# aynik/carta1

Measured on AMD Instinct MI355X. Metric: atrac1_stereo_frames_per_s_encode, higher is better.
Workload: dtype f32+f64

## Files before the change

### carta1_amd/capi.py

```python
import ctypes as C
import os

HERE = os.path.dirname(os.path.abspath(__file__))
LIB_PATH = os.environ.get('C1_LIB') or os.path.join(HERE, 'lib', 'libcarta1_hip.so')

FRAME = 512
UNIT_BYTES = 212
SIGNAL_WHITE = 0
SIGNAL_PINK_BURSTS = 1
SIGNAL_MIXED = 2
SIGNAL_PARTIALS = 3


class Carta1Error(RuntimeError):
    def __init__(self, code, message):
        super().__init__('carta1_hip error %d: %s' % (code, message))
        self.code = code


class Tables(C.Structure):
    _fields_ = [('scale_factors', C.c_double * 64), ('window_short', C.c_double * 32),
                ('mdct_fwd64', C.c_double * 32), ('mdct_fwd256', C.c_double * 128),
                ('mdct_fwd512', C.c_double * 256), ('mdct_inv64', C.c_double * 32),
                ('mdct_inv256', C.c_double * 128), ('mdct_inv512', C.c_double * 256),
# ... 16 lines not shown
    'c1_ctx_destroy': (C.c_int, [C.c_void_p]),
    'c1_ctx_synchronize': (C.c_int, [C.c_void_p]),
    'c1_ctx_set_profiling': (C.c_int, [C.c_void_p, C.c_int]),
    'c1_ctx_kernel_ms': (C.c_int, [C.c_void_p, C.c_char_p, C.POINTER(C.c_double), C.POINTER(C.c_int)]),
    'c1_ctx_set_speculation': (C.c_int, [C.c_void_p, C.c_int]),
    'c1_ctx_set_decode_precision': (C.c_int, [C.c_void_p, C.c_int]),
    'c1_ctx_speculation_stats': (C.c_int, [C.c_void_p, C.POINTER(C.c_uint64), C.POINTER(C.c_uint64), C.c_int]),
    'c1_ctx_speculation_deferred': (C.c_int, [C.c_void_p, C.POINTER(C.c_uint64)]),
    'c1_ctx_quantization_stats': (C.c_int, [C.c_void_p, C.POINTER(C.c_uint64), C.POINTER(C.c_uint64)]),
    'c1_encode_device': (C.c_int, [C.c_void_p, C.POINTER(C.c_void_p), C.c_int, C.c_int64, C.c_int,
                                   C.POINTER(EncodeOptions), C.c_void_p]),
    'c1_encode_batch': (C.c_int, [C.c_void_p, C.POINTER(C.c_void_p), C.c_int, C.c_int64, C.c_int,
                                  C.POINTER(EncodeOptions), C.c_void_p]),
    'c1_encode_batch_multi': (C.c_int, [C.POINTER(C.c_int), C.c_int, C.POINTER(C.c_void_p), C.c_int, C.c_int64, C.c_int,
                                        C.POINTER(EncodeOptions), C.c_void_p]),
    'c1_decode_batch_multi': (C.c_int, [C.POINTER(C.c_int), C.c_int, C.c_void_p, C.c_int, C.c_int64, C.c_int,
                                        C.POINTER(C.c_void_p)]),
    'c1_decode_device': (C.c_int, [C.c_void_p, C.c_void_p, C.c_int, C.c_int64, C.c_int, C.POINTER(C.c_void_p)]),
    'c1_decode_batch': (C.c_int, [C.c_void_p, C.c_void_p, C.c_int, C.c_int64, C.c_int, C.POINTER(C.c_void_p)]),
    'c1_enc_stream_create': (C.c_int, [C.c_void_p, C.c_int, C.POINTER(EncodeOptions), C.POINTER(C.c_void_p)]),
    'c1_enc_stream_push': (C.c_int, [C.c_void_p, C.POINTER(C.c_void_p), C.c_int64, C.c_void_p]),
    'c1_enc_stream_destroy': (C.c_int, [C.c_void_p]),
    'c1_enc_stream_set_options': (C.c_int, [C.c_void_p, C.POINTER(EncodeOptions)]),
    'c1_dec_stream_create': (C.c_int, [C.c_void_p, C.c_int, C.POINTER(C.c_void_p)]),
    'c1_dec_stream_push': (C.c_int, [C.c_void_p, C.c_void_p, C.c_int64, C.POINTER(C.c_void_p)]),
    'c1_dec_stream_destroy': (C.c_int, [C.c_void_p]),
    'c1_generate_device': (C.c_int, [C.c_void_p, C.c_int, C.c_uint32, C.c_int64, C.c_void_p]),
    'c1_pcm_from_int_device': (C.c_int, [C.c_void_p, C.c_void_p, C.c_int, C.c_int, C.c_int64, C.POINTER(C.c_void_p)]),
    'c1_pcm_to_int16_device': (C.c_int, [C.c_void_p, C.POINTER(C.c_void_p), C.c_int, C.c_int64, C.c_void_p]),
    'c1_host_alloc': (C.c_int, [C.c_size_t, C.POINTER(C.c_void_p)]),
    'c1_host_free': (C.c_int, [C.c_void_p]),
    'c1_table_fast_paths': (C.c_int, [C.POINTER(C.c_int), C.POINTER(C.c_int)]),
    'c1_alloc_rank_form': (C.c_int, [C.POINTER(EncodeOptions), C.POINTER(C.c_int), C.POINTER(C.c_int)]),
    'c1_encode_wav_batch': (C.c_int, [C.c_void_p, C.c_void_p, C.c_int, C.c_int, C.c_int64, C.POINTER(EncodeOptions), C.c_void_p]),
    'c1_decode_wav16_batch': (C.c_int, [C.c_void_p, C.c_void_p, C.c_int, C.c_int64, C.c_void_p]),
    'c1_aea_header': (C.c_int, [C.c_char_p, C.c_uint32, C.c_int, C.c_void_p]),
    'c1_encode_stages_device': (C.c_int, [C.c_void_p, C.POINTER(C.c_void_p), C.c_int, C.c_int64, C.c_int,
                                          C.POINTER(EncodeOptions), C.c_void_p, C.c_void_p, C.c_void_p,
                                          C.c_void_p]),
    'c1_detect_stages_device': (C.c_int, [C.c_void_p, C.POINTER(C.c_void_p), C.c_int, C.c_int64, C.c_int,
                                          C.POINTER(EncodeOptions), C.c_void_p, C.c_void_p]),
    'c1_libm_device': (C.c_int, [C.c_void_p, C.c_int, C.c_void_p, C.c_void_p, C.c_int64]),
    'c1_detect_scores_device': (C.c_int, [C.c_void_p, C.POINTER(C.c_void_p), C.c_int, C.c_int64, C.c_int,
                                          C.POINTER(EncodeOptions), C.c_int, C.c_void_p, C.c_void_p, C.c_void_p]),
    'c1_detect_spec_mags_device': (C.c_int, [C.c_void_p, C.POINTER(C.c_void_p), C.c_int, C.c_int64, C.c_int, C.c_void_p, C.c_void_p]),
    'c1_log2f_error_device': (C.c_int, [C.c_void_p, C.c_uint32, C.c_uint64, C.POINTER(C.c_double)]),
    'c1_ctx_detection_stats': (C.c_int, [C.c_void_p, C.POINTER(C.c_uint64), C.POINTER(C.c_uint64)]),
    'c1_alloc_bounds_device': (C.c_int, [C.c_void_p, C.c_void_p, C.c_int64, C.c_void_p, C.c_void_p]),
    'c1_spec_stages_device': (C.c_int, [C.c_void_p, C.POINTER(C.c_void_p), C.c_int, C.c_int64, C.c_int,
                                        C.POINTER(EncodeOptions), C.c_void_p, C.c_void_p, C.c_void_p]),
    'c1_quantize': (C.c_int, [C.c_void_p, C.c_void_p, C.c_int, C.c_int, C.c_int, C.c_void_p]),
    'c1_dequantize': (C.c_int, [C.c_void_p, C.c_void_p, C.c_int, C.c_int, C.c_int, C.c_void_p]),
    'c1_fft': (C.c_int, [C.c_void_p, C.c_void_p, C.c_void_p, C.c_int, C.c_void_p]),
    'c1_qmf_analysis_batch': (C.c_int, [C.c_void_p, C.c_void_p, C.c_int64, C.c_int, C.c_void_p]),
    'c1_mdct_batch': (C.c_int, [C.c_void_p, C.c_void_p, C.c_int64, C.c_int, C.c_void_p, C.c_void_p, C.c_void_p]),
    'c1_unpack_units': (C.c_int, [C.c_void_p, C.c_void_p, C.c_int64, C.c_void_p, C.c_void_p, C.c_void_p, C.c_void_p, C.c_void_p]),
    'c1_dequantize_frames': (C.c_int, [C.c_void_p, C.c_int64, C.c_void_p, C.c_void_p, C.c_void_p, C.c_void_p, C.c_void_p, C.c_void_p]),
    'c1_imdct_batch': (C.c_int, [C.c_void_p, C.c_void_p, C.c_int64, C.c_int, C.c_void_p, C.c_void_p]),
    'c1_qmf_synthesis_batch': (C.c_int, [C.c_void_p, C.c_void_p, C.c_int64, C.c_int, C.c_void_p]),
    'c1_select_block_modes': (C.c_int, [C.c_void_p, C.c_void_p, C.c_int64, C.c_int, C.c_double, C.c_void_p]),
    'c1_quantize_frames': (C.c_int, [C.c_void_p, C.c_void_p, C.c_int64, C.c_void_p, C.c_void_p, C.c_void_p, C.c_void_p,
                                     C.c_void_p, C.c_void_p]),
    'c1_pack_units': (C.c_int, [C.c_void_p, C.c_int64, C.c_void_p, C.c_void_p, C.c_void_p, C.c_void_p, C.c_void_p, C.c_void_p]),
    'c1_decode_fields_device': (C.c_int, [C.c_void_p, C.c_int, C.c_int64, C.c_int, C.c_void_p, C.c_void_p, C.c_void_p, C.c_void_p,
                                          C.c_void_p, C.POINTER(C.c_void_p)]),
    'c1_decode_fields_batch': (C.c_int, [C.c_void_p, C.c_int, C.c_int64, C.c_int, C.c_void_p, C.c_void_p, C.c_void_p, C.c_void_p,
# ... 55 lines not shown
```

### carta1_amd/csrc/c1_api.hip

```cpp
#include <algorithm>
#include <cmath>
#include <cstdarg>
#include <cstdio>
#include <cstdlib>
#include <cstring>
#include <map>
#include <memory>
#include <atomic>
#include <mutex>
#include <string>
#include <thread>
#include <vector>

#include "c1_internal.h"
#include "c1_detect_bound.h"

#pragma clang fp contract(off)

namespace {

#include "c1_default_tables.inc"

thread_local std::string g_error;
int fail(int code, const char *fmt, ...) {
  char buf[512];
  va_list ap;
  va_start(ap, fmt);
  vsnprintf(buf, sizeof buf, fmt, ap);
  va_end(ap);
  g_error = buf;
  return code;
}
#define HIP_TRY(expr)                                                                        \
  do {                                                                                       \
    hipError_t e_ = (expr);                                                                  \
    if (e_ != hipSuccess) return fail(C1_ERR_HIP, "%s: %s", #expr, hipGetErrorString(e_)); \
  } while (0)

// ... 242 lines not shown
      const double dbits = (double)(b1 - b0);
      pri[s * 15 + wl] = (float)(d->biased[s] * ddf / dbits);
      uniq.push_back(pri[s * 15 + wl]);
    }
  std::sort(uniq.begin(), uniq.end());
  uniq.erase(std::unique(uniq.begin(), uniq.end()), uniq.end());
  for (int s = 1; s < 64; s++)
    for (int wl = 0; wl < 15; wl++) {
      const auto it = std::lower_bound(uniq.begin(), uniq.end(), pri[s * 15 + wl]);
      d->rank[s * 16 + wl] = (uint16_t)(1 + (it - uniq.begin()));
    }
  d->rank_affine = 0;
  {
    std::vector<int> order;
    for (int s = 1; s < 64; s++)
      for (int wl = 0; wl < 15; wl++) order.push_back(s * 16 + wl);
    std::sort(order.begin(), order.end(), [&](int x, int y) { return d->rank[x] < d->rank[y]; });
    for (int A = 1; A <= 12 && !d->rank_affine; A++)
      for (int B = 1; B <= 36 && !d->rank_affine; B++)
        for (int C = -2 * B; C <= 2 * B && !d->rank_affine; C++) {
          auto key = [&](int idx) { const int s = idx >> 4, wl = idx & 15; return wl == 0 ? A * s + C : A * s - B * wl - B; };
          bool ok = true;
          int lo = key(order[0]), hi = lo;
          for (size_t i = 1; i < order.size() && ok; i++) {
            const int k0 = key(order[i - 1]), k1 = key(order[i]);
            const bool req = d->rank[order[i]] == d->rank[order[i - 1]];
            if (req ? (k1 != k0) : !(k1 > k0)) ok = false;
            lo = std::min(lo, k1); hi = std::max(hi, k1);
          }
          if (ok && hi - lo + 1 < 1023) {
            d->rank_affine = 1; d->rank_a = A; d->rank_b = B; d->rank_c = C; d->rank_off = 1 - lo;
          }
        }
  }
  return C1_OK;
}

constexpr int kTotals = 8;
constexpr int64_t kSpecMinUnits = 64;
constexpr int kListHead = 8;
constexpr int64_t kMaxChunkFrames = (int64_t)1 << 27;

struct Timing {
  hipEvent_t start, stop;
  int kind;
};
enum { K_ANALYSIS = 0, K_ALLOCATE, K_PACK, K_DECODE, K_REDO, K_PACK_UNITS, K_DECODE_FIELDS, K_KINDS };
const char *const kKindNames[K_KINDS] = {"analysis", "allocate", "pack", "decode", "redo", "pack_units", "decode_fields"};

}

struct c1_ctx {
  std::recursive_mutex mu;
  int device = 0;
  hipStream_t stream = nullptr;
  bool own_stream = false;
  C1DevTables *d_tables = nullptr;
  C1DevEncOpts *d_opts = nullptr;
  c1_encode_options last_opts;
  bool have_opts = false;
  int64_t ws_units = 0;
  float *d_coefs[2] = {nullptr, nullptr};
  uint8_t *d_side[2] = {nullptr, nullptr};
  uint8_t *d_alloc[2] = {nullptr, nullptr};
  uint8_t *d_cand[2] = {nullptr, nullptr};
  uint32_t *d_work[2] = {nullptr, nullptr};
// ... 467 lines not shown
  if (!tables) { g_tables_custom = false; g_tables_gen++; return C1_OK; }
  const double *p = reinterpret_cast<const double *>(tables);
  for (size_t i = 0; i < sizeof(c1_tables) / sizeof(double); i++)
    if (!std::isfinite(p[i])) return fail(C1_ERR_ARG, "table entry %zu is not finite", i);
  g_tables = *tables;
  g_tables_custom = true;
  g_tables_gen++;
  return C1_OK;
}

int c1_table_fast_paths(int *scale_factor_bits, int *dequant_reciprocal) {
  c1_tables t;
  {
    std::lock_guard<std::mutex> lock(g_tables_mutex);
    if (g_tables_custom) t = g_tables; else default_tables(&t);
  }
  std::unique_ptr<C1DevTables> d(new C1DevTables);
  build_device_tables(t, d.get());
  if (scale_factor_bits) *scale_factor_bits = d->sf_fast;
  if (dequant_reciprocal) *dequant_reciprocal = d->dq_fast + d->dq_step;
  return C1_OK;
}

int c1_alloc_rank_form(const c1_encode_options *opts, int *affine, int *coef) {
  if (!opts) return fail(C1_ERR_ARG, "opts is NULL");
  std::unique_ptr<C1DevEncOpts> d(new C1DevEncOpts);
  const int rc = build_table_fields(*opts, d.get());
  if (rc) return rc;
  if (affine) *affine = d->rank_affine;
  if (coef) { coef[0] = d->rank_a; coef[1] = d->rank_b; coef[2] = d->rank_c; coef[3] = d->rank_off; }
  return C1_OK;
}

int c1_default_encode_options(c1_encode_options *out) {
  if (!out) return fail(C1_ERR_ARG, "out is NULL");
  memset(out, 0, sizeof *out);
  c1_tables t;
  {
    std::lock_guard<std::mutex> lock(g_tables_mutex);
    if (g_tables_custom) t = g_tables; else default_tables(&t);
  }
  memcpy(out->biased_scale_factors, t.scale_factors, sizeof out->biased_scale_factors);
  out->transient_threshold = 1.0;
  out->fixed_block_modes[0] = out->fixed_block_modes[1] = out->fixed_block_modes[2] = -1;
  return C1_OK;
}

int c1_ctx_create(int device, void *hip_stream, c1_ctx **out) {
  if (!out) return fail(C1_ERR_ARG, "out is NULL");
  *out = nullptr;
  int n = 0;
  const hipError_t e = hipGetDeviceCount(&n);
  if (e != hipSuccess || n == 0)
    return fail(C1_ERR_NO_DEVICE, "no HIP device available (%s); this library has no CPU path",
                e != hipSuccess ? hipGetErrorString(e) : "device count is 0");
  if (device < 0 || device >= n) return fail(C1_ERR_ARG, "device %d out of range (0..%d)", device, n - 1);
  HIP_TRY(hipSetDevice(device));
  c1_ctx *ctx = new c1_ctx();
  ctx->device = device;
  if (hip_stream) ctx->stream = (hipStream_t)hip_stream;
  else {
    const hipError_t se = hipStreamCreateWithFlags(&ctx->stream, hipStreamNonBlocking);
    if (se != hipSuccess) { delete ctx; return fail(C1_ERR_HIP, "hipStreamCreate: %s", hipGetErrorString(se)); }
    ctx->own_stream = true;
  }
  c1_tables t;
// ... 1930 lines not shown
```

### carta1_amd/csrc/c1_internal.h

```cpp
#pragma once

#include <hip/hip_runtime.h>
#include <stdint.h>
#include <stdlib.h>

#include "../../include/carta1_hip.h"

struct C1DevTables {
  double tap_e[24];
  double tap_o[24];
  double window[32];
  double mdct_fwd64[32];
  double mdct_fwd256[128];
  double mdct_fwd512[256];
  double mdct_inv64[32];
  double mdct_inv256[128];
  double mdct_inv512[256];
  double fft_tw[256][2];
  double scale_factors[64];
  double norm[64 * 16];
  double log1p10;
  uint32_t sf_m1, sf_m2;
  int32_t sf_fast;
  int32_t dq_fast;
  int32_t dq_step;
  double inv_range[16];
  float tap32[24];
  float tap_pair[26][2];
  float win32[32];
  float pre32_64[16][2];
  float pre32_256[64][2];
  float pre32_512[128][2];
  float r4b[4][3][2];
  float r4c[16][3][2];
  float r2d[64][2];
  float norm32[64 * 16];
  float inv32_64[16][2], inv32_256[64][2], inv32_512[128][2];
  float tw32[256][2];
  float spec_cz[4], spec_cw[4], spec_cl[4];
  float spec_cz_short[4], spec_cw_short[4], spec_cl_short[4];
  float spec_eabs;
  float det_ck[4];
  float det_eabs;
  int32_t spec_ok;
};

struct C1DevEncOpts {
  double biased[64];
  double threshold;
  int32_t modes[3];
  int32_t pad_;
  uint16_t rank[64 * 16];
  int32_t rank_affine, rank_a, rank_b, rank_c, rank_off;
  float la_slope, la_off;
  int32_t alloc_no_tonal;
};

constexpr int kRunFrames = 16;
constexpr int kRunFramesDecode = 64;
constexpr int kRunFramesLong = 64;
constexpr int kSideBytes = 64;
constexpr int kAllocBytes = 32;
constexpr int kCandidateBytes = 8 * 8 + 8 * 32 + 8 * 8;
constexpr int kCandLbOffset = 8 * 8 + 8 * 32;
constexpr int kEpsFloats = 4;
constexpr uint32_t kEpsFlagSfOpen = 1u;
constexpr uint32_t kEpsFlagExact = 2u;
constexpr int kSpecCheckFrames = 16;

struct C1EncodeLaunch {
  const float *pcm[C1_MAX_CHANNELS];
  int channels;
  int64_t frames;
  int halo_frames;
  const C1DevTables *tables;
  const C1DevEncOpts *opts;
  float *coefs;
  uint8_t *side;
  uint8_t *alloc;
  uint8_t *cand;
  uint32_t *work_list;
  uint32_t *work_count;
  uint32_t *sel_list;
  float *bands;
  float *mags;
  float *mag_bounds;
  uint8_t *units;
  float *eps;
  uint32_t *redo_list;
// ... 116 lines not shown
```

### carta1_amd/csrc/c1_k_allocate.hip

```cpp
#include "c1_device.h"

namespace {

constexpr int kHeapSlotsPerLane = 52 + 1;
constexpr uint32_t kLow = 0x1FFFFFu;
constexpr uint32_t kSentinel = 52u;
constexpr int kCandBytes = kCandidateBytes;
constexpr double kAlive = -1.0;

__device__ __forceinline__ uint32_t heap_entry(uint32_t rank, int size, int s, int wl, int b) {
  return (rank << 21) | ((uint32_t)size << 16) | ((uint32_t)s << 10) | ((uint32_t)wl << 6) | (uint32_t)b;
}

__device__ __forceinline__ void heap_sift_down(uint32_t *hp, int sentinel, int i, uint32_t v, uint32_t el,
                                               uint32_t er, bool active) {
  const uint32_t vmax = v | kLow;
  for (;;) {
    const uint32_t m = max(el | kLow, vmax);
    const bool take_r = er > m;
    const bool take_l = !take_r && el > vmax;
    const bool moved = active && (take_r || take_l);
    if (active) hp[i * 64] = moved ? (take_r ? er : el) : v;
    active = moved;
    if (__builtin_amdgcn_ballot_w64(active) == 0) break;
    i = moved ? 2 * i + 1 + (take_r ? 1 : 0) : i;
    const int l = 2 * i + 1;
    const uint32_t *src = hp + min(l, sentinel - 1) * 64;
    el = l < sentinel ? src[0] : 0u;
    er = src[64];
  }
}

__device__ __forceinline__ void run_candidate(uint32_t *hp, int n, const uint32_t (&sf)[13], const C1DevEncOpts *O,
                                              bool live, uint64_t &res0, uint64_t &res1, uint64_t &res2,
                                              uint64_t &res3, double &total) {
  const __attribute__((address_space(4))) uint16_t *rank_t = (const __attribute__((address_space(4))) uint16_t *)O->rank;
  const __attribute__((address_space(4))) double *biased = (const __attribute__((address_space(4))) double *)O->biased;
  const bool affine = O->rank_affine != 0;
  const int ka = O->rank_a, kb = O->rank_b, kc = O->rank_c, koff = O->rank_off;
  const int nkb = -kb, kc_off = kc + koff;
  auto rank_of = [&](int s, int wl) -> uint32_t {
    if (affine) return (uint32_t)(wl == 0 ? __mul24(ka, s) + kc_off : __mul24(ka, s) + koff + __mul24(nkb, wl + 1));
    return rank_t[s * 16 + (wl & 15)];
  };
  int remaining = 212 * 8 - 40 - 10 * n;
  int hs = 0;
#pragma unroll
  for (int b = 0; b < 52; b++) {
    if (b < n) {
      const int s = (sf[b >> 2] >> ((b & 3) * 8)) & 63;
      hp[hs * 64] = heap_entry(rank_of(s, 0), kSpecs[b], s, 0, b);
      hs += (s != 0 && live) ? 1 : 0;
    }
  }
  for (int k = hs; k < kHeapSlotsPerLane; k++) hp[k * 64] = kSentinel;
  for (int i = (hs >> 1) - 1; i >= 0; i--) {
    const int l = 2 * i + 1;
    heap_sift_down(hp, 52, i, hp[i * 64], hp[l * 64], hp[(l + 1) * 64], true);
  }
  uint32_t r0 = hp[0], r1 = hp[64], r2 = hp[128];
  bool run = remaining >= 4 && hs > 0;
  while (__builtin_amdgcn_ballot_w64(run) != 0) {
    const uint32_t top = r0;
    const int wl = (top >> 6) & 15, size = (top >> 16) & 31, s = (top >> 10) & 63;
    const int cost = size << (wl == 0 ? 1 : 0);
    const bool fits = cost <= remaining;
    const int nxt = wl + (fits ? 1 : 0);
    const bool leaves = run && (!fits || nxt >= 15);
    const uint32_t upd = (top & ~((0x3FFu << 21) | (15u << 6))) | ((uint32_t)nxt << 6);
    uint32_t v = upd | (rank_of(s, nxt) << 21);
    if (__builtin_amdgcn_ballot_w64(leaves) != 0) {
      const int li = hs - 1;
      const uint32_t deep = hp[(li > 3 ? li : 3) * 64];
      const uint32_t last = li == 0 ? r0 : (li == 1 ? r1 : (li == 2 ? r2 : deep));
      if (leaves) {
        v = last;
        hs = li;
        if (li > 2) hp[li * 64] = upd;
        r0 = li == 0 ? upd : r0; r1 = li == 1 ? upd : r1; r2 = li == 2 ? upd : r2;
      }
    }
    if (run) remaining -= fits ? cost : 0;
    const bool sift = run && hs > 0;
    const uint32_t vmax = v | kLow;
    const bool tr0 = r2 > max(r1 | kLow, vmax);
    const bool tl0 = !tr0 && r1 > vmax;
    const bool mv0 = sift && (tr0 || tl0);
    if (sift) r0 = mv0 ? (tr0 ? r2 : r1) : v;
    {
      const int i1 = tr0 ? 2 : 1;
      const uint32_t *src = hp + (2 * i1 + 1) * 64;
      const uint32_t el = src[0], er = src[64];
      const uint32_t g0 = src[(2 * i1 + 2) * 64], g1 = src[(2 * i1 + 3) * 64], g2 = src[(2 * i1 + 4) * 64], g3 = src[(2 * i1 + 5) * 64];
      const bool tr1 = er > max(el | kLow, vmax);
      const bool tl1 = !tr1 && el > vmax;
      const bool mv1 = mv0 && (tr1 || tl1);
      const uint32_t val = mv1 ? (tr1 ? er : el) : v;
      if (mv0) { if (tr0) r2 = val; else r1 = val; }
      {
        const int i2 = 2 * i1 + 1 + (tr1 ? 1 : 0);
        const uint32_t c0 = tr1 ? g2 : g0, c1 = tr1 ? g3 : g1;
        const bool tr2 = c1 > max(c0 | kLow, vmax);
        const bool tl2 = !tr2 && c0 > vmax;
        const bool mv2 = mv1 && (tr2 || tl2);
        if (mv1) hp[i2 * 64] = mv2 ? (tr2 ? c1 : c0) : v;
        if (__builtin_amdgcn_ballot_w64(mv2) != 0) {
          const int i3 = 2 * i2 + 1 + (tr2 ? 1 : 0);
          const uint32_t *s3 = hp + (2 * i3 + 1) * 64;
          const uint32_t d0 = s3[0], d1 = s3[64];
          const int q = 4 * i3 + 3;
          const uint32_t h0 = hp[min(q, 52) * 64], h1 = hp[min(q + 1, 52) * 64], h2 = hp[min(q + 2, 52) * 64], h3 = hp[min(q + 3, 52) * 64];
          const bool tr3 = d1 > max(d0 | kLow, vmax);
          const bool tl3 = !tr3 && d0 > vmax;
          const bool mv3 = mv2 && (tr3 || tl3);
          if (mv2) hp[i3 * 64] = mv3 ? (tr3 ? d1 : d0) : v;
          const int i4 = 2 * i3 + 1 + (tr3 ? 1 : 0);
          const uint32_t e0 = tr3 ? h2 : h0, e1 = tr3 ? h3 : h1;
          const bool tr4 = e1 > max(e0 | kLow, vmax);
          const bool tl4 = !tr4 && e0 > vmax;
          const bool mv4 = mv3 && (tr4 || tl4);
          if (mv3) hp[i4 * 64] = mv4 ? (tr4 ? e1 : e0) : v;
          if (mv4) hp[(2 * i4 + 1 + (tr4 ? 1 : 0)) * 64] = v;
        }
      }
    }
    run = run && remaining >= 4 && hs > 0;
  }
  hp[0] = r0; hp[64] = r1; hp[128] = r2;
  {
    uint8_t *hb = reinterpret_cast<uint8_t *>(hp);
#pragma unroll
    for (int k = 0; k < 52; k++) hb[k * 256 + 3] = 0;
#pragma unroll
    for (int k0 = 0; k0 < 52; k0 += 8) {
      uint32_t e[8];
#pragma unroll
      for (int j = 0; j < 8; j++) if (k0 + j < 52) e[j] = hp[(k0 + j) * 64];
#pragma unroll
      for (int j = 0; j < 8; j++) if (k0 + j < 52) hb[(e[j] & 63u) * 256 + 3] = (uint8_t)((e[j] >> 6) & 15u);
    }
    uint32_t d[8];
#pragma unroll
    for (int i = 0; i < 8; i++) {
      d[i] = 0;
#pragma unroll
      for (int j = 0; j < 8; j++) if (8 * i + j < 52) d[i] |= (hp[(8 * i + j) * 64] >> 24) << (4 * j);
    }
    res0 = (uint64_t)d[0] | ((uint64_t)d[1] << 32); res1 = (uint64_t)d[2] | ((uint64_t)d[3] << 32);
    res2 = (uint64_t)d[4] | ((uint64_t)d[5] << 32); res3 = (uint64_t)d[6] | ((uint64_t)d[7] << 32);
  }
  total = 0.0;
#pragma unroll
  for (int b = 0; b < 52; b++) {
    const int s = (sf[b >> 2] >> ((b & 3) * 8)) & 63;
    const uint64_t word = b < 16 ? res0 : (b < 32 ? res1 : (b < 48 ? res2 : res3));
    const int wl = (int)((word >> ((b & 15) * 4)) & 15);
    const int size = kSpecs[b];
    const double bs = biased[s];
    if (b >= n || wl == 0) {
      total += s != 0 ? (double)f32(bs * 2.0 * (double)size) : 0.0;
    } else if (s != 0) {
      const double ip2 = __hiloint2double((1023 - wl_bits(wl)) << 20, 0);
      total += bs * ip2 * (double)size;
    }
  }
}

__device__ __forceinline__ void load_sfi(const uint8_t *side, int64_t unit, uint32_t (&sf)[13]) {
  const uint4 *src = reinterpret_cast<const uint4 *>(side + unit * kSideBytes);
  const uint4 a = src[0], b = src[1], c = src[2];
  const uint32_t d = reinterpret_cast<const uint32_t *>(src)[12];
  sf[0] = a.x; sf[1] = a.y; sf[2] = a.z; sf[3] = a.w; sf[4] = b.x; sf[5] = b.y; sf[6] = b.z; sf[7] = b.w;
  sf[8] = c.x; sf[9] = c.y; sf[10] = c.z; sf[11] = c.w; sf[12] = d;
}

__device__ __forceinline__ void store_candidate(uint8_t *cand, int64_t unit, int c, double total, uint64_t r0,
                                                uint64_t r1, uint64_t r2, uint64_t r3) {
  uint8_t *base = cand + unit * kCandBytes;
  reinterpret_cast<double *>(base)[c] = total;
  uint64_t *dst = reinterpret_cast<uint64_t *>(base + 64 + c * 32);
  dst[0] = r0; dst[1] = r1; dst[2] = r2; dst[3] = r3;
}

__device__ __forceinline__ bool getenv_no_tonal(const C1DevEncOpts *O) { return O->alloc_no_tonal != 0; }

__global__ __launch_bounds__(C1_WAVE, 3) void k_alloc_first(C1EncodeLaunch L) {
  __shared__ uint32_t heap[kHeapSlotsPerLane * 64];
  const C1DevEncOpts *O = L.opts;
  const __attribute__((address_space(4))) double *biased = (const __attribute__((address_space(4))) double *)O->biased;
  const int lane = threadIdx.x;
  const bool listed = L.unit_list != nullptr;
  const int64_t units_total = listed ? (int64_t)*L.unit_count : L.frames * L.channels;
  for (int64_t pos0 = (int64_t)blockIdx.x * 64; pos0 < units_total; pos0 += (int64_t)gridDim.x * 64) {
  const int64_t pos = pos0 + lane;
  const bool live = pos < units_total;
  const int64_t unit = listed ? (int64_t)L.unit_list[live ? pos : 0] : pos;
  uint32_t sf[13];
  load_sfi(L.side, live ? unit : 0, sf);
  bool tonal = false;
  {
    float n_coef = 0.0f, s_la = 0.0f;
#pragma unroll
    for (int b = 0; b < 52; b++) {
      const int s = (sf[b >> 2] >> ((b & 3) * 8)) & 63;
      const float w = s != 0 ? (float)kSpecs[b] : 0.0f;
      n_coef += w;
      s_la = __builtin_fmaf(w, (float)s, s_la);
    }
    const float la_sum = __builtin_fmaf(O->la_slope, s_la, O->la_off * n_coef);
    const float t_est = 1.442695f * n_coef * __builtin_amdgcn_exp2f((la_sum - 1136.0f) / n_coef);
    float t6f = 0.0f;
#pragma unroll
    for (int b = 48; b < 52; b++) {
      const int s = (sf[b >> 2] >> ((b & 3) * 8)) & 63;
      const float bs = (float)biased[s];
      t6f += s != 0 ? bs * (2.0f * (float)kSpecs[b]) : 0.0f;
    }
    const bool mine = n_coef > 0.0f && t6f < 0.35f * t_est && !getenv_no_tonal(O);
    tonal = 2 * __popcll(__builtin_amdgcn_ballot_w64(live && mine)) > __popcll(__builtin_amdgcn_ballot_w64(live));
  }
  uint64_t r0, r1, r2, r3;
  double total;
  run_candidate(heap + lane, 52, sf, O, live && !tonal, r0, r1, r2, r3, total);
  uint32_t survivors = 0;
  {
    double t0 = 0, t1 = 0, t2 = 0, t3 = 0, t4 = 0, t5 = 0, t6 = 0;
#pragma unroll
    for (int b = 20; b < 52; b++) {
      const int s = (sf[b >> 2] >> ((b & 3) * 8)) & 63;
      const double bs = biased[s];
      const double z = s != 0 ? (double)f32(bs * 2.0 * (double)kSpecs[b]) : 0.0;
      t0 += z;
      if (b >= 28) t1 += z;
      if (b >= 32) t2 += z;
      if (b >= 36) t3 += z;
      if (b >= 40) t4 += z;
      if (b >= 44) t5 += z;
      if (b >= 48) t6 += z;
    }
    const bool finite = total < __builtin_huge_val();
    survivors = (!(finite && t0 > total) ? 1u : 0u) | (!(finite && t1 > total) ? 2u : 0u) |
                (!(finite && t2 > total) ? 4u : 0u) | (!(finite && t3 > total) ? 8u : 0u) |
                (!(finite && t4 > total) ? 16u : 0u) | (!(finite && t5 > total) ? 32u : 0u) |
                (!(finite && t6 > total) ? 64u : 0u);
  }
  if (tonal) survivors = 0xffu;
  const bool finite52 = total < __builtin_huge_val();
  if (live && survivors == 0) {
    uint64_t *dst = reinterpret_cast<uint64_t *>(L.alloc + unit * kAllocBytes);
    if (finite52) { dst[0] = r0; dst[1] = r1; dst[2] = r2; dst[3] = r3 | (7ull << 60); }
    else { dst[0] = 0; dst[1] = 0; dst[2] = 0; dst[3] = 1ull << 59; }
  } else if (live) {
    uint8_t *base = L.cand + unit * kCandBytes;
    double *tot = reinterpret_cast<double *>(base);
#pragma unroll
    for (int c = 0; c < 7; c++) tot[c] = ((survivors >> c) & 1u) ? kAlive : __builtin_huge_val();
    if (tonal) tot[7] = kAlive;
    else store_candidate(L.cand, unit, 7, finite52 ? total : __builtin_huge_val(), r0, r1, r2, r3);
  }
  const uint64_t sel_mask = __builtin_amdgcn_ballot_w64(live && survivors != 0);
  uint32_t sel_base = 0;
  if (lane == 0 && sel_mask != 0) sel_base = atomicAdd(L.work_count + 1, (uint32_t)__popcll(sel_mask));
  sel_base = (uint32_t)__builtin_amdgcn_readfirstlane((int)sel_base);
  if (live && survivors != 0) L.sel_list[sel_base + (uint32_t)__popcll(sel_mask & ((1ull << lane) - 1ull))] = (uint32_t)unit;
  }
}

typedef _Float16 h2 __attribute__((ext_vector_type(2)));
constexpr int kSpecsHost[52] = {8, 8, 8, 8, 4, 4, 4, 4, 8, 8, 8, 8, 6, 6, 6, 6, 6, 6, 6, 6, 6, 6, 6, 6, 7, 7, 7, 7, 9, 9, 9, 9, 10, 10, 10, 10,
                                12, 12, 12, 12, 12, 12, 12, 12, 20, 20, 20, 20, 20, 20, 20, 20};
__global__ __launch_bounds__(256) void k_alloc_bound(C1EncodeLaunch L) {
  __shared__ double biased_s[64];
  const C1DevEncOpts *O = L.opts;
  if (threadIdx.x < 64) biased_s[threadIdx.x] = threadIdx.x == 0 ? 0.0 : ((const __attribute__((address_space(4))) double *)O->biased)[threadIdx.x];
  __syncthreads();
  const float la_slope = O->la_slope, la_off = O->la_off;
  const int lane = threadIdx.x & 63;
  const uint32_t count = L.work_count[1];
  for (uint32_t pos0 = blockIdx.x * 256u; pos0 < count; pos0 += gridDim.x * 256u) {
    const uint32_t pos = pos0 + threadIdx.x;
    const bool live = pos < count;
    const int64_t unit = live ? (int64_t)L.sel_list[pos] : (int64_t)L.sel_list[0];
    uint32_t sf[13];
    load_sfi(L.side, unit, sf);
    uint8_t *base = L.cand + unit * kCandBytes;
    double *tot = reinterpret_cast<double *>(base);
    double *lb = reinterpret_cast<double *>(base + kCandLbOffset);
    const double t52 = tot[7];
    const double best = t52 == kAlive ? __builtin_huge_val() : t52;
    int smin = 64, smax = 0;
#pragma unroll
    for (int b = 0; b < 52; b++) {
      const int s = (sf[b >> 2] >> ((b & 3) * 8)) & 63;
      if (s != 0) { smin = s < smin ? s : smin; smax = s > smax ? s : smax; }
    }
    h2 sp[26];
#pragma unroll
    for (int k = 0; k < 26; k++) {
      const int s0 = (sf[(2 * k) >> 2] >> (((2 * k) & 3) * 8)) & 63, s1 = (sf[(2 * k + 1) >> 2] >> (((2 * k + 1) & 3) * 8)) & 63;
      sp[k] = h2{s0 != 0 ? (_Float16)s0 : (_Float16)-1000.0f, s1 != 0 ? (_Float16)s1 : (_Float16)-1000.0f};
    }
    const h2 slope2 = h2{(_Float16)la_slope, (_Float16)la_slope};
    float x_prev = 0.0f;
// ... 52 lines not shown
        else {
          lb[c] = bound;
          if (bound < lb_star || c_star < 0) { lb_star = bound; c_star = c; }
        }
        x_prev = x; have_prev = true;
      }
    }
    const bool has = live && c_star >= 0;
    const uint64_t m = __builtin_amdgcn_ballot_w64(has);
    uint32_t at = 0;
    if (lane == 0 && m != 0) at = atomicAdd(L.work_count, (uint32_t)__popcll(m));
    at = (uint32_t)__builtin_amdgcn_readfirstlane((int)at);
    if (has) L.work_list[at + (uint32_t)__popcll(m & ((1ull << lane) - 1ull))] = ((uint32_t)unit << 3) | (uint32_t)c_star;
  }
}

template <bool FIRST_ROUND>
__global__ __launch_bounds__(C1_WAVE, 3) void k_alloc_rest(C1EncodeLaunch L, const uint32_t *__restrict__ list, const uint32_t *__restrict__ list_count,
                                                           uint32_t *__restrict__ list2) {
  __shared__ uint32_t heap[kHeapSlotsPerLane * 64];
  const C1DevEncOpts *O = L.opts;
  const int lane = threadIdx.x;
  const uint32_t count = *list_count;
  for (uint32_t base = blockIdx.x * 64u; base < count; base += gridDim.x * 64u) {
    const uint32_t idx = base + lane;
    const bool live = idx < count;
    const uint32_t item = live ? list[idx] : 0u;
    const int64_t unit = item >> 3;
    const int c = item & 7;
    uint32_t sf[13];
    load_sfi(L.side, unit, sf);
    uint64_t r0, r1, r2, r3;
    double total;
    run_candidate(heap + lane, bfu_amount(c), sf, O, live, r0, r1, r2, r3, total);
    total = total < __builtin_huge_val() ? total : __builtin_huge_val();
    if (live) store_candidate(L.cand, unit, c, total, r0, r1, r2, r3);
    if constexpr (FIRST_ROUND) {
      uint8_t *cbase = L.cand + unit * kCandBytes;
      double *tot = reinterpret_cast<double *>(cbase);
      const double *lb = reinterpret_cast<const double *>(cbase + kCandLbOffset);
      uint32_t keep = 0;
      if (live) {
        const double t52 = tot[7];
        const double best = (c == 7 || t52 == kAlive || total < t52) ? total : t52;
#pragma unroll
        for (int k = 0; k < 8; k++) {
          if (k != c && tot[k] == kAlive) {
            if (lb[k] > best) tot[k] = __builtin_huge_val();
            else keep |= 1u << k;
          }
        }
      }
      const int mine = __popc(keep);
      const int scan = wave_inclusive_scan(mine);
      const int wave_total = __builtin_amdgcn_readlane(scan, 63);
      uint32_t at = 0;
      if (lane == 0 && wave_total > 0) at = atomicAdd(L.work_count + 2, (uint32_t)wave_total);
      at = (uint32_t)__builtin_amdgcn_readfirstlane((int)at) + (uint32_t)(scan - mine);
      for (int k = 0; k < 8; k++)
        if ((keep >> k) & 1u) list2[at++] = ((uint32_t)unit << 3) | (uint32_t)k;
    }
  }
}

__global__ __launch_bounds__(256) void k_alloc_select(C1EncodeLaunch L) {
  const int64_t count = (int64_t)L.work_count[1];
  for (int64_t pos = (int64_t)blockIdx.x * 256 + threadIdx.x; pos < count; pos += (int64_t)gridDim.x * 256) {
// ... 75 lines not shown
```

### include/carta1_hip.h

```cpp
#ifndef CARTA1_HIP_H
#define CARTA1_HIP_H

#include <stddef.h>
#include <stdint.h>

#ifdef __cplusplus
extern "C" {
#endif

#define C1_FRAME_SAMPLES 512
#define C1_UNIT_BYTES 212
#define C1_MAX_CHANNELS 2
#define C1_ABI_VERSION 3

enum {
  C1_OK = 0,
  C1_ERR_ARG = 1,
  C1_ERR_NO_DEVICE = 2,
  C1_ERR_HIP = 3,
  C1_ERR_STATE = 4
};

typedef struct c1_tables {
  double scale_factors[64];
  double window_short[32];
  double mdct_fwd64[32];
  double mdct_fwd256[128];
  double mdct_fwd512[256];
  double mdct_inv64[32];
  double mdct_inv256[128];
  double mdct_inv512[256];
  double fft_w[8][2];
  double log1p_10;
} c1_tables;

typedef struct c1_encode_options {
  double biased_scale_factors[64];
  double transient_threshold;
  int32_t fixed_block_modes[3];
  int32_t reserved;
} c1_encode_options;

typedef struct c1_ctx c1_ctx;

int c1_abi_version(void);
const char *c1_last_error(void);
int c1_device_count(int *count);
int c1_get_default_tables(c1_tables *out);
int c1_set_tables(const c1_tables *tables);
int c1_default_encode_options(c1_encode_options *out);
int c1_table_fast_paths(int *scale_factor_bits, int *dequant_reciprocal);
int c1_alloc_rank_form(const c1_encode_options *opts, int *affine, int *coef);

int c1_ctx_create(int device, void *hip_stream , c1_ctx **out);
int c1_ctx_destroy(c1_ctx *ctx);
int c1_ctx_synchronize(c1_ctx *ctx);
int c1_ctx_set_profiling(c1_ctx *ctx, int enabled);
int c1_ctx_kernel_ms(c1_ctx *ctx, const char *name, double *ms, int *launches);

int c1_ctx_set_speculation(c1_ctx *ctx, int mode);
int c1_ctx_speculation_stats(c1_ctx *ctx, uint64_t *units, uint64_t *redone, int reset);
int c1_ctx_speculation_deferred(c1_ctx *ctx, uint64_t *units);
int c1_ctx_quantization_stats(c1_ctx *ctx, uint64_t *units, uint64_t *repacked);
int c1_ctx_detection_stats(c1_ctx *ctx, uint64_t *units, uint64_t *rechecked);

int c1_ctx_set_decode_precision(c1_ctx *ctx, int binary32);


int c1_encode_device(c1_ctx *ctx, const float *const *pcm, int channels, int64_t frames,
                     int halo_frames, const c1_encode_options *opts, uint8_t *units);
int c1_encode_batch(c1_ctx *ctx, const float *const *pcm, int channels, int64_t frames,
                    int halo_frames, const c1_encode_options *opts, uint8_t *units);

int c1_encode_batch_multi(const int *devices, int n_devices, const float *const *pcm, int channels, int64_t frames,
                          int halo_frames, const c1_encode_options *opts, uint8_t *units);
int c1_decode_batch_multi(const int *devices, int n_devices, const uint8_t *units, int channels, int64_t frames,
                          int halo_units, float *const *pcm);

int c1_host_alloc(size_t bytes, void **out);
int c1_host_free(void *p);

int c1_decode_device(c1_ctx *ctx, const uint8_t *units, int channels, int64_t frames,
                     int halo_units, float *const *pcm);
int c1_decode_batch(c1_ctx *ctx, const uint8_t *units, int channels, int64_t frames,
                    int halo_units, float *const *pcm);
// ... 94 lines not shown
```

Measured before the change: 179.6 million.

## Precompute distortion tables and affine rank steps for allocation heap kernels

Adds host-built per-size distortion tables (zero-bit cost and coded cost whose exponent is decremented per word length) and precomputed affine rank step increments, so the heap loop advances an entry by a single add instead of recomputing the rank. The totals and lower-bound sums are fused into one pass, the tonal estimate uses packed-byte SAD integer sums, and the heap sift drops some clamped loads. Tables are validated on the host and fall back to the direct path when an exact bit match cannot be guaranteed. The aim is fewer ALU and FP64 operations and fewer constant-memory lookups in the allocation kernels, at the cost of more code and template variants.

```diff
diff --git a/carta1_amd/capi.py b/carta1_amd/capi.py
--- a/carta1_amd/capi.py
+++ b/carta1_amd/capi.py
@@ -72,6 +72,7 @@
     'c1_host_free': (C.c_int, [C.c_void_p]),
     'c1_table_fast_paths': (C.c_int, [C.POINTER(C.c_int), C.POINTER(C.c_int)]),
     'c1_alloc_rank_form': (C.c_int, [C.POINTER(EncodeOptions), C.POINTER(C.c_int), C.POINTER(C.c_int)]),
+    'c1_alloc_tables': (C.c_int, [C.POINTER(EncodeOptions), C.POINTER(C.c_int), C.c_void_p, C.c_void_p, C.POINTER(C.c_int), C.c_void_p]),
     'c1_encode_wav_batch': (C.c_int, [C.c_void_p, C.c_void_p, C.c_int, C.c_int, C.c_int64, C.POINTER(EncodeOptions), C.c_void_p]),
     'c1_decode_wav16_batch': (C.c_int, [C.c_void_p, C.c_void_p, C.c_int, C.c_int64, C.c_void_p]),
     'c1_aea_header': (C.c_int, [C.c_char_p, C.c_uint32, C.c_int, C.c_void_p]),
diff --git a/carta1_amd/csrc/c1_api.hip b/carta1_amd/csrc/c1_api.hip
--- a/carta1_amd/csrc/c1_api.hip
+++ b/carta1_amd/csrc/c1_api.hip
@@ -4,6 +4,7 @@
 #include <cstdio>
 #include <cstdlib>
 #include <cstring>
+#include <limits>
 #include <map>
 #include <memory>
 #include <atomic>
@@ -312,6 +313,45 @@
             d->rank_affine = 1; d->rank_a = A; d->rank_b = B; d->rank_c = C; d->rank_off = 1 - lo;
           }
         }
+  }
+  if (d->rank_affine) {
+    const int A = d->rank_a, B = d->rank_b, C = d->rank_c, off = d->rank_off;
+    auto rk = [&](int s, int wl) { return wl == 0 ? A * s + C + off : A * s + off - B * (wl + 1); };
+    auto entry = [&](int s, int wl) { return ((uint32_t)rk(s, wl) << 21) | ((uint32_t)s << 10) | ((uint32_t)wl << 6); };
+    d->rank_step0 = (1u << 6) + ((uint32_t)(-2 * B - C) << 21);
+    d->rank_step = (1u << 6) - ((uint32_t)B << 21);
+    bool ok = true;
+    for (int s = 1; s < 64 && ok; s++)
+      for (int wl = 0; wl < 15 && ok; wl++) {
+        if (rk(s, wl) < 1 || rk(s, wl) > 1022) ok = false;
+        if (wl < 14 && entry(s, wl) + (wl == 0 ? d->rank_step0 : d->rank_step) != entry(s, wl + 1)) ok = false;
+      }
+    if (!ok) { d->rank_affine = 0; d->rank_step0 = d->rank_step = 0; }
+  }
+  {
+    bool ok = true;
+    for (int c = 0; c < 8; c++) {
+      const double size = (double)kDistSizes[c];
+      for (int s = 0; s < 64; s++) {
+        const double bs = d->biased[s];
+        const double zb = s != 0 ? (double)(float)(bs * 2.0 * size) : 0.0;
+        const double cs = bs * size;
+        d->dist[c][s][0] = zb;
+        d->dist[c][s][1] = cs;
+        if (s == 0) continue;
+        if (!(zb >= (double)std::numeric_limits<float>::min())) ok = false;
+        uint64_t u;
+        memcpy(&u, &cs, sizeof u);
+        for (int wl = 1; wl <= 15; wl++) {
+          const int bits = wl + 1;
+          const double want = bs * std::ldexp(1.0, -bits) * size;
+          if ((int)((u >> 52) & 0x7ff) <= bits || (int)((u >> 52) & 0x7ff) == 0x7ff) { ok = false; continue; }
+          const uint64_t v = u - ((uint64_t)bits << 52);
+          if (memcmp(&v, &want, sizeof v) != 0) ok = false;
+        }
+      }
+    }
+    d->dist_tables = (ok && !getenv("C1_NO_DIST_TABLES")) ? 1 : 0;
   }
   return C1_OK;
 }
@@ -845,6 +885,24 @@
   return C1_OK;
 }
 
+int c1_alloc_tables(const c1_encode_options *opts, int *affine, uint32_t *steps, uint16_t *rank, int *dist_ok, double *dist) {
+  if (!opts) return fail(C1_ERR_ARG, "opts is NULL");
+  std::unique_ptr<C1DevEncOpts> d(new C1DevEncOpts);
+  const int rc = build_table_fields(*opts, d.get());
+  if (rc) return rc;
+  if (affine) *affine = d->rank_affine;
+  if (steps) { steps[0] = d->rank_step0; steps[1] = d->rank_step; }
+  if (rank) {
+    for (int s = 0; s < 64; s++)
+      for (int wl = 0; wl < 16; wl++)
+        rank[s * 16 + wl] = !d->rank_affine ? d->rank[s * 16 + wl]
+                            : (uint16_t)(wl == 0 ? d->rank_a * s + d->rank_c + d->rank_off : d->rank_a * s + d->rank_off - d->rank_b * (wl + 1));
+  }
+  if (dist_ok) *dist_ok = d->dist_tables;
+  if (dist) memcpy(dist, d->dist, sizeof d->dist);
+  return C1_OK;
+}
+
 int c1_default_encode_options(c1_encode_options *out) {
   if (!out) return fail(C1_ERR_ARG, "out is NULL");
   memset(out, 0, sizeof *out);
diff --git a/carta1_amd/csrc/c1_internal.h b/carta1_amd/csrc/c1_internal.h
--- a/carta1_amd/csrc/c1_internal.h
+++ b/carta1_amd/csrc/c1_internal.h
@@ -54,7 +54,11 @@
   int32_t rank_affine, rank_a, rank_b, rank_c, rank_off;
   float la_slope, la_off;
   int32_t alloc_no_tonal;
-};
+  uint32_t rank_step0, rank_step;
+  int32_t dist_tables;
+  alignas(16) double dist[8][64][2];
+};
+constexpr int kDistSizes[8] = {4, 6, 7, 8, 9, 10, 12, 20};
 
 constexpr int kRunFrames = 16;
 constexpr int kRunFramesDecode = 64;
diff --git a/carta1_amd/csrc/c1_k_allocate.hip b/carta1_amd/csrc/c1_k_allocate.hip
--- a/carta1_amd/csrc/c1_k_allocate.hip
+++ b/carta1_amd/csrc/c1_k_allocate.hip
@@ -31,27 +31,43 @@
   }
 }
 
-__device__ __forceinline__ void run_candidate(uint32_t *hp, int n, const uint32_t (&sf)[13], const C1DevEncOpts *O,
-                                              bool live, uint64_t &res0, uint64_t &res1, uint64_t &res2,
-                                              uint64_t &res3, double &total) {
+constexpr int kSpecsHost[52] = {8, 8, 8, 8, 4, 4, 4, 4, 8, 8, 8, 8, 6, 6, 6, 6, 6, 6, 6, 6, 6, 6, 6, 6, 7, 7, 7, 7, 9, 9, 9, 9, 10, 10, 10, 10,
+                                12, 12, 12, 12, 12, 12, 12, 12, 20, 20, 20, 20, 20, 20, 20, 20};
+constexpr int dist_class(int size) {
+  for (int c = 0; c < 8; c++) if (kDistSizes[c] == size) return c;
+  return -1;
+}
+constexpr bool sizes_come_in_fours() {
+  for (int b = 0; b < 52; b++) if (kSpecsHost[b] != kSpecsHost[b & ~3]) return false;
+  return true;
+}
+static_assert(sizes_come_in_fours(), "the four BFUs whose indices share a dword share a size");
+static_assert(dist_class(4) == 0 && dist_class(20) == 7 && dist_class(kSpecsHost[24]) == 2, "every BFU size has its row of the distortion tables");
+
+__device__ __forceinline__ void reopen(uint32_t (&sf)[13]) {
+#pragma unroll
+  for (int i = 0; i < 13; i++) asm volatile("" : "+v"(sf[i]));
+}
+
+template <bool AFFINE>
+__device__ __forceinline__ void heap_phase(uint32_t *hp, int n, const uint32_t (&sf)[13], const C1DevEncOpts *O, bool live) {
   const __attribute__((address_space(4))) uint16_t *rank_t = (const __attribute__((address_space(4))) uint16_t *)O->rank;
-  const __attribute__((address_space(4))) double *biased = (const __attribute__((address_space(4))) double *)O->biased;
-  const bool affine = O->rank_affine != 0;
-  const int ka = O->rank_a, kb = O->rank_b, kc = O->rank_c, koff = O->rank_off;
-  const int nkb = -kb, kc_off = kc + koff;
-  auto rank_of = [&](int s, int wl) -> uint32_t {
-    if (affine) return (uint32_t)(wl == 0 ? __mul24(ka, s) + kc_off : __mul24(ka, s) + koff + __mul24(nkb, wl + 1));
-    return rank_t[s * 16 + (wl & 15)];
-  };
+  const uint32_t mul0 = ((uint32_t)O->rank_a << 11) | 1u, add0 = (uint32_t)(O->rank_c + O->rank_off) << 11;
+  const uint32_t step0 = O->rank_step0, step = O->rank_step;
   int remaining = 212 * 8 - 40 - 10 * n;
   int hs = 0;
 #pragma unroll
-  for (int b = 0; b < 52; b++) {
+  for (int b0 = 0; b0 < 52; b0 += 13) if (own_block()) {
+#pragma unroll
+  for (int b = b0; b < b0 + 13; b++) {
     if (b < n) {
       const int s = (sf[b >> 2] >> ((b & 3) * 8)) & 63;
-      hp[hs * 64] = heap_entry(rank_of(s, 0), kSpecs[b], s, 0, b);
+      const uint32_t fixed = ((uint32_t)kSpecsHost[b] << 16) | (uint32_t)b;
+      if constexpr (AFFINE) hp[hs * 64] = ((__umul24(mul0, (uint32_t)s) + add0) << 10) | fixed;
+      else hp[hs * 64] = ((uint32_t)rank_t[s * 16] << 21) | ((uint32_t)s << 10) | fixed;
       hs += (s != 0 && live) ? 1 : 0;
     }
+  }
   }
   for (int k = hs; k < kHeapSlotsPerLane; k++) hp[k * 64] = kSentinel;
   for (int i = (hs >> 1) - 1; i >= 0; i--) {
@@ -62,13 +78,24 @@
   bool run = remaining >= 4 && hs > 0;
   while (__builtin_amdgcn_ballot_w64(run) != 0) {
     const uint32_t top = r0;
-    const int wl = (top >> 6) & 15, size = (top >> 16) & 31, s = (top >> 10) & 63;
-    const int cost = size << (wl == 0 ? 1 : 0);
+    const bool wl0 = (top & (15u << 6)) == 0;
+    const int size = (top >> 16) & 31;
+    const int cost = size << (wl0 ? 1 : 0);
     const bool fits = cost <= remaining;
-    const int nxt = wl + (fits ? 1 : 0);
-    const bool leaves = run && (!fits || nxt >= 15);
-    const uint32_t upd = (top & ~((0x3FFu << 21) | (15u << 6))) | ((uint32_t)nxt << 6);
-    uint32_t v = upd | (rank_of(s, nxt) << 21);
+    uint32_t v, upd;
+    bool last_wl;
+    if constexpr (AFFINE) {
+      v = top + (wl0 ? step0 : step);
+      upd = (fits ? v : top) & kLow;
+      last_wl = (v & (15u << 6)) == (15u << 6);
+    } else {
+      const int wl = (top >> 6) & 15, s = (top >> 10) & 63;
+      const int nxt = wl + (fits ? 1 : 0);
+      upd = (top & ~((0x3FFu << 21) | (15u << 6))) | ((uint32_t)nxt << 6);
+      v = upd | ((uint32_t)rank_t[s * 16 + (nxt & 15)] << 21);
+      last_wl = nxt >= 15;
+    }
+    const bool leaves = run && (!fits || last_wl);
     if (__builtin_amdgcn_ballot_w64(leaves) != 0) {
       const int li = hs - 1;
       const uint32_t deep = hp[(li > 3 ? li : 3) * 64];
@@ -108,17 +135,19 @@
           const int i3 = 2 * i2 + 1 + (tr2 ? 1 : 0);
           const uint32_t *s3 = hp + (2 * i3 + 1) * 64;
           const uint32_t d0 = s3[0], d1 = s3[64];
-          const int q = 4 * i3 + 3;
-          const uint32_t h0 = hp[min(q, 52) * 64], h1 = hp[min(q + 1, 52) * 64], h2 = hp[min(q + 2, 52) * 64], h3 = hp[min(q + 3, 52) * 64];
+          const bool far = i3 >= 12;
+          const uint32_t *s4 = hp + min(4 * i3 + 3, 49) * 64;
+          const uint32_t h0 = s4[0], h1 = s4[64], h2 = s4[128], h3 = s4[192];
           const bool tr3 = d1 > max(d0 | kLow, vmax);
           const bool tl3 = !tr3 && d0 > vmax;
           const bool mv3 = mv2 && (tr3 || tl3);
           if (mv2) hp[i3 * 64] = mv3 ? (tr3 ? d1 : d0) : v;
           const int i4 = 2 * i3 + 1 + (tr3 ? 1 : 0);
-          const uint32_t e0 = tr3 ? h2 : h0, e1 = tr3 ? h3 : h1;
+          const bool upper = tr3 || far;
+          const uint32_t e0 = upper ? h2 : h0, e1 = upper ? h3 : h1;
           const bool tr4 = e1 > max(e0 | kLow, vmax);
           const bool tl4 = !tr4 && e0 > vmax;
-          const bool mv4 = mv3 && (tr4 || tl4);
+          const bool mv4 = mv3 && i4 < 26 && (tr4 || tl4);
           if (mv3) hp[i4 * 64] = mv4 ? (tr4 ? e1 : e0) : v;
           if (mv4) hp[(2 * i4 + 1 + (tr4 ? 1 : 0)) * 64] = v;
         }
@@ -127,43 +156,103 @@
     run = run && remaining >= 4 && hs > 0;
   }
   hp[0] = r0; hp[64] = r1; hp[128] = r2;
-  {
-    uint8_t *hb = reinterpret_cast<uint8_t *>(hp);
-#pragma unroll
-    for (int k = 0; k < 52; k++) hb[k * 256 + 3] = 0;
-#pragma unroll
-    for (int k0 = 0; k0 < 52; k0 += 8) {
-      uint32_t e[8];
-#pragma unroll
-      for (int j = 0; j < 8; j++) if (k0 + j < 52) e[j] = hp[(k0 + j) * 64];
-#pragma unroll
-      for (int j = 0; j < 8; j++) if (k0 + j < 52) hb[(e[j] & 63u) * 256 + 3] = (uint8_t)((e[j] >> 6) & 15u);
-    }
-    uint32_t d[8];
-#pragma unroll
-    for (int i = 0; i < 8; i++) {
-      d[i] = 0;
-#pragma unroll
-      for (int j = 0; j < 8; j++) if (8 * i + j < 52) d[i] |= (hp[(8 * i + j) * 64] >> 24) << (4 * j);
-    }
-    res0 = (uint64_t)d[0] | ((uint64_t)d[1] << 32); res1 = (uint64_t)d[2] | ((uint64_t)d[3] << 32);
-    res2 = (uint64_t)d[4] | ((uint64_t)d[5] << 32); res3 = (uint64_t)d[6] | ((uint64_t)d[7] << 32);
-  }
+}
+
+template <bool BOUND>
+__device__ __forceinline__ void totals_tabled(int n, const uint32_t (&sf)[13], const C1DevEncOpts *O, uint64_t res0, uint64_t res1,
+                                              uint64_t res2, uint64_t res3, double &total, double (&lbs)[7]) {
+  typedef double d2 __attribute__((ext_vector_type(2)));
+  const __attribute__((address_space(4))) d2 *dist = (const __attribute__((address_space(4))) d2 *)O->dist;
   total = 0.0;
 #pragma unroll
-  for (int b = 0; b < 52; b++) {
+  for (int c = 0; c < 7; c++) lbs[c] = 0.0;
+#pragma unroll
+  for (int b0 = 0; b0 < 52; b0 += 13) if (own_block()) {
+#pragma unroll
+  for (int b = b0; b < b0 + 13; b++) {
     const int s = (sf[b >> 2] >> ((b & 3) * 8)) & 63;
     const uint64_t word = b < 16 ? res0 : (b < 32 ? res1 : (b < 48 ? res2 : res3));
     const int wl = (int)((word >> ((b & 15) * 4)) & 15);
-    const int size = kSpecs[b];
+    const d2 zc = dist[dist_class(kSpecsHost[b]) * 64 + s];
+    const double coded = __hiloint2double(__double2hiint(zc.y) - ((wl + 1) << 20), __double2loint(zc.y));
+    total += (b >= n || wl == 0) ? zc.x : coded;
+    if constexpr (BOUND) {
+      if (b >= 20) lbs[0] += zc.x;
+      if (b >= 28) lbs[1] += zc.x;
+      if (b >= 32) lbs[2] += zc.x;
+      if (b >= 36) lbs[3] += zc.x;
+      if (b >= 40) lbs[4] += zc.x;
+      if (b >= 44) lbs[5] += zc.x;
+      if (b >= 48) lbs[6] += zc.x;
+    }
+  }
+  }
+}
+
+template <bool BOUND>
+__device__ __forceinline__ void totals_direct(int n, const uint32_t (&sf)[13], const C1DevEncOpts *O, uint64_t res0, uint64_t res1,
+                                              uint64_t res2, uint64_t res3, double &total, double (&lbs)[7]) {
+  const __attribute__((address_space(4))) double *biased = (const __attribute__((address_space(4))) double *)O->biased;
+  total = 0.0;
+#pragma unroll
+  for (int c = 0; c < 7; c++) lbs[c] = 0.0;
+#pragma unroll
+  for (int b0 = 0; b0 < 52; b0 += 13) if (own_block()) {
+#pragma unroll
+  for (int b = b0; b < b0 + 13; b++) {
+    const int s = (sf[b >> 2] >> ((b & 3) * 8)) & 63;
+    const uint64_t word = b < 16 ? res0 : (b < 32 ? res1 : (b < 48 ? res2 : res3));
+    const int wl = (int)((word >> ((b & 15) * 4)) & 15);
+    const int size = kSpecsHost[b];
     const double bs = biased[s];
-    if (b >= n || wl == 0) {
-      total += s != 0 ? (double)f32(bs * 2.0 * (double)size) : 0.0;
-    } else if (s != 0) {
-      const double ip2 = __hiloint2double((1023 - wl_bits(wl)) << 20, 0);
-      total += bs * ip2 * (double)size;
-    }
-  }
+    const double z = s != 0 ? (double)f32(bs * 2.0 * (double)size) : 0.0;
+    const double ip2 = __hiloint2double((1023 - wl_bits(wl)) << 20, 0);
+    const double coded = s != 0 ? bs * ip2 * (double)size : 0.0;
+    total += (b >= n || wl == 0) ? z : coded;
+    if constexpr (BOUND) {
+      if (b >= 20) lbs[0] += z;
+      if (b >= 28) lbs[1] += z;
+      if (b >= 32) lbs[2] += z;
+      if (b >= 36) lbs[3] += z;
+      if (b >= 40) lbs[4] += z;
+      if (b >= 44) lbs[5] += z;
+      if (b >= 48) lbs[6] += z;
+    }
+  }
+  }
+}
+
+template <bool BOUND>
+__device__ __forceinline__ void run_candidate(uint32_t *hp, int n, uint32_t (&sf)[13], const C1DevEncOpts *O,
+                                              bool live, uint64_t &res0, uint64_t &res1, uint64_t &res2,
+                                              uint64_t &res3, double &total, double (&lbs)[7]) {
+  if (O->rank_affine != 0) heap_phase<true>(hp, n, sf, O, live);
+  else heap_phase<false>(hp, n, sf, O, live);
+  {
+    uint8_t *hb = reinterpret_cast<uint8_t *>(hp);
+#pragma unroll
+    for (int k = 0; k < 52; k++) hb[k * 256 + 3] = 0;
+#pragma unroll
+    for (int k0 = 0; k0 < 52; k0 += 8) {
+      uint32_t e[8];
+#pragma unroll
+      for (int j = 0; j < 8; j++) if (k0 + j < 52) e[j] = hp[(k0 + j) * 64];
+#pragma unroll
+      for (int j = 0; j < 8; j++) if (k0 + j < 52) hb[(e[j] & 63u) * 256 + 3] = (uint8_t)((e[j] >> 6) & 15u);
+    }
+    uint32_t d[8];
+#pragma unroll
+    for (int i = 0; i < 8; i++) {
+      d[i] = 0;
+#pragma unroll
+      for (int j = 0; j < 8; j++) if (8 * i + j < 52) d[i] |= (hp[(8 * i + j) * 64] >> 24) << (4 * j);
+    }
+    res0 = (uint64_t)d[0] | ((uint64_t)d[1] << 32); res1 = (uint64_t)d[2] | ((uint64_t)d[3] << 32);
+    res2 = (uint64_t)d[4] | ((uint64_t)d[5] << 32); res3 = (uint64_t)d[6] | ((uint64_t)d[7] << 32);
+  }
+  reopen(sf);
+  if (O->dist_tables != 0) totals_tabled<BOUND>(n, sf, O, res0, res1, res2, res3, total, lbs);
+  else totals_direct<BOUND>(n, sf, O, res0, res1, res2, res3, total, lbs);
 }
 
 __device__ __forceinline__ void load_sfi(const uint8_t *side, int64_t unit, uint32_t (&sf)[13]) {
@@ -199,14 +288,15 @@
   load_sfi(L.side, live ? unit : 0, sf);
   bool tonal = false;
   {
-    float n_coef = 0.0f, s_la = 0.0f;
-#pragma unroll
-    for (int b = 0; b < 52; b++) {
-      const int s = (sf[b >> 2] >> ((b & 3) * 8)) & 63;
-      const float w = s != 0 ? (float)kSpecs[b] : 0.0f;
-      n_coef += w;
-      s_la = __builtin_fmaf(w, (float)s, s_la);
-    }
+    uint32_t n_int = 0, s_int = 0;
+#pragma unroll
+    for (int g = 0; g < 13; g++) {
+      const uint32_t x = sf[g] & 0x3F3F3F3Fu;
+      const uint32_t nz = ((x + 0x3F3F3F3Fu) >> 6) & 0x01010101u;
+      n_int = __umul24(__builtin_amdgcn_sad_u8(nz, 0u, 0u), (uint32_t)kSpecsHost[4 * g]) + n_int;
+      s_int = __umul24(__builtin_amdgcn_sad_u8(x, 0u, 0u), (uint32_t)kSpecsHost[4 * g]) + s_int;
+    }
+    const float n_coef = (float)n_int, s_la = (float)s_int;
     const float la_sum = __builtin_fmaf(O->la_slope, s_la, O->la_off * n_coef);
     const float t_est = 1.442695f * n_coef * __builtin_amdgcn_exp2f((la_sum - 1136.0f) / n_coef);
     float t6f = 0.0f;
@@ -214,30 +304,19 @@
     for (int b = 48; b < 52; b++) {
       const int s = (sf[b >> 2] >> ((b & 3) * 8)) & 63;
       const float bs = (float)biased[s];
-      t6f += s != 0 ? bs * (2.0f * (float)kSpecs[b]) : 0.0f;
+      t6f += s != 0 ? bs * (2.0f * (float)kSpecsHost[b]) : 0.0f;
     }
     const bool mine = n_coef > 0.0f && t6f < 0.35f * t_est && !getenv_no_tonal(O);
     tonal = 2 * __popcll(__builtin_amdgcn_ballot_w64(live && mine)) > __popcll(__builtin_amdgcn_ballot_w64(live));
   }
   uint64_t r0, r1, r2, r3;
   double total;
-  run_candidate(heap + lane, 52, sf, O, live && !tonal, r0, r1, r2, r3, total);
+  double lbs[7];
+  reopen(sf);
+  run_candidate<true>(heap + lane, 52, sf, O, live && !tonal, r0, r1, r2, r3, total, lbs);
   uint32_t survivors = 0;
   {
-    double t0 = 0, t1 = 0, t2 = 0, t3 = 0, t4 = 0, t5 = 0, t6 = 0;
-#pragma unroll
-    for (int b = 20; b < 52; b++) {
-      const int s = (sf[b >> 2] >> ((b & 3) * 8)) & 63;
-      const double bs = biased[s];
-      const double z = s != 0 ? (double)f32(bs * 2.0 * (double)kSpecs[b]) : 0.0;
-      t0 += z;
-      if (b >= 28) t1 += z;
-      if (b >= 32) t2 += z;
-      if (b >= 36) t3 += z;
-      if (b >= 40) t4 += z;
-      if (b >= 44) t5 += z;
-      if (b >= 48) t6 += z;
-    }
+    const double t0 = lbs[0], t1 = lbs[1], t2 = lbs[2], t3 = lbs[3], t4 = lbs[4], t5 = lbs[5], t6 = lbs[6];
     const bool finite = total < __builtin_huge_val();
     survivors = (!(finite && t0 > total) ? 1u : 0u) | (!(finite && t1 > total) ? 2u : 0u) |
                 (!(finite && t2 > total) ? 4u : 0u) | (!(finite && t3 > total) ? 8u : 0u) |
@@ -267,8 +346,6 @@
 }
 
 typedef _Float16 h2 __attribute__((ext_vector_type(2)));
-constexpr int kSpecsHost[52] = {8, 8, 8, 8, 4, 4, 4, 4, 8, 8, 8, 8, 6, 6, 6, 6, 6, 6, 6, 6, 6, 6, 6, 6, 7, 7, 7, 7, 9, 9, 9, 9, 10, 10, 10, 10,
-                                12, 12, 12, 12, 12, 12, 12, 12, 20, 20, 20, 20, 20, 20, 20, 20};
 __global__ __launch_bounds__(256) void k_alloc_bound(C1EncodeLaunch L) {
   __shared__ double biased_s[64];
   const C1DevEncOpts *O = L.opts;
@@ -387,7 +464,8 @@
     load_sfi(L.side, unit, sf);
     uint64_t r0, r1, r2, r3;
     double total;
-    run_candidate(heap + lane, bfu_amount(c), sf, O, live, r0, r1, r2, r3, total);
+    double unused[7];
+    run_candidate<false>(heap + lane, bfu_amount(c), sf, O, live, r0, r1, r2, r3, total, unused);
     total = total < __builtin_huge_val() ? total : __builtin_huge_val();
     if (live) store_candidate(L.cand, unit, c, total, r0, r1, r2, r3);
     if constexpr (FIRST_ROUND) {
diff --git a/include/carta1_hip.h b/include/carta1_hip.h
--- a/include/carta1_hip.h
+++ b/include/carta1_hip.h
@@ -51,6 +51,7 @@
 int c1_default_encode_options(c1_encode_options *out);
 int c1_table_fast_paths(int *scale_factor_bits, int *dequant_reciprocal);
 int c1_alloc_rank_form(const c1_encode_options *opts, int *affine, int *coef);
+int c1_alloc_tables(const c1_encode_options *opts, int *affine, uint32_t *steps, uint16_t *rank, int *dist_ok, double *dist);
 
 int c1_ctx_create(int device, void *hip_stream , c1_ctx **out);
 int c1_ctx_destroy(c1_ctx *ctx);
```

Result: faster. 185.3 million, median of 6 (+3.2%).
